# nyu-systems/Grendel-GS

Measured on NVIDIA H100. Metric: train-step Gaussians/s (preprocess+forward+loss+backward), higher is better.
Workload: dtype f32

## Files before the change

### grendel-gs_b200/csrc/binning.cu

```cuda
#include <cub/cub.cuh>

#include "common.cuh"
#include <atomic>
#include <cfloat>
#include <mutex>

#define BIN_THREADS 256

GS_D uint32_t count_local_tiles(int i, int W, int H, const float *__restrict__ means2D, const int32_t *__restrict__ radii,
                                const uint8_t *__restrict__ compute_locally, const GsViews &views) {
    const int gx = (W + GS_BLOCK_X - 1) / GS_BLOCK_X, gy = (H + GS_BLOCK_Y - 1) / GS_BLOCK_Y;
    const int r = radii[i];
    uint32_t n = 0;
    if (r > 0) {
        const float2 m = *reinterpret_cast<const float2 *>(means2D + 2 * i);
        int x0, y0, x1, y1;
        gs_get_rect(m.x, m.y, r, gx, gy, x0, y0, x1, y1);
        const uint8_t *mask = compute_locally + (size_t)gs_view_of(views, i) * views.T;
        for (int y = y0; y < y1; y++) {
            const uint8_t *row = mask + y * gx;
            for (int x = x0; x < x1; x++) n += row[x] ? 1u : 0u;
        }
    }
    return n;
}

__global__ void __launch_bounds__(BIN_THREADS)
k_count_tiles(int P, int W, int H, const float *__restrict__ means2D, const float *__restrict__ conic_opacity,
              const float *__restrict__ rgb, const float *__restrict__ depths, const int32_t *__restrict__ radii,
              const uint8_t *__restrict__ compute_locally, uint32_t *__restrict__ touched,
              uint32_t *__restrict__ depth_key, uint32_t *__restrict__ index, float *__restrict__ rec, int no_cull,
              unsigned long long *__restrict__ total64, const GsViews views) {
    const int i = blockIdx.x * BIN_THREADS + threadIdx.x;
    const bool valid = i < P;
    const uint32_t my_n = valid ? count_local_tiles(i, W, H, means2D, radii, compute_locally, views) : 0u;
    {
        __shared__ uint32_t s_sum[BIN_THREADS / 32];
        const uint32_t wsum = __reduce_add_sync(0xffffffffu, my_n);
        if ((threadIdx.x & 31) == 0) s_sum[threadIdx.x >> 5] = wsum;
        __syncthreads();
        if (threadIdx.x == 0) {
            unsigned long long t = 0ull;
#pragma unroll
            for (int w = 0; w < BIN_THREADS / 32; w++) t += s_sum[w];
            if (t) atomicAdd(total64, t);
        }
    }
    if (!valid) return;
    const uint32_t n = my_n;
    const float2 m = *reinterpret_cast<const float2 *>(means2D + 2 * i);
    touched[i] = n;
    depth_key[i] = n > 0 ? __float_as_uint(depths[i]) : 0xffffffffu;
    index[i] = (uint32_t)i;
    float4 r0 = make_float4(0.f, 0.f, 0.f, 0.f), r1 = r0, r2 = r0;
    if (n > 0) {
        const float4 co = *reinterpret_cast<const float4 *>(conic_opacity + 4 * i);
        const float thr = -logf(255.0f * fmaxf(co.w, 1e-30f));
        const float t = -2.f * thr;
        const float bb = co.y * co.y, bb_err = __fmaf_rn(co.y, co.y, -bb);
        const float det = __fmaf_rn(co.x, co.z, -bb) - bb_err;
        float ex = -1.f, ey = -1.f;
        if (t >= 0.f) {
            if (!no_cull && det >= FLT_MIN && co.x > 0.f && co.z > 0.f) {
                ex = sqrtf(t * co.z / det) * 1.02f + 0.5f;
                ey = sqrtf(t * co.x / det) * 1.02f + 0.5f;
            } else {
                ex = ey = 3.0e38f;
            }
        }
        r0 = make_float4(m.x, m.y, -0.5f * co.x, -co.y);
        r1 = make_float4(-0.5f * co.z, co.w, thr, rgb[3 * i]);
        r2 = make_float4(rgb[3 * i + 1], rgb[3 * i + 2], ex, ey);
    }
    float4 *o = reinterpret_cast<float4 *>(rec + (size_t)GS_REC_FLOATS * i);
    o[0] = r0; o[1] = r1; o[2] = r2;
}

struct TouchedInDepthOrder {
    const uint32_t *order, *touched;
    __host__ __device__ __forceinline__ uint32_t operator()(int s) const { return touched[order[s]]; }
};

template <bool DET>
__global__ void __launch_bounds__(BIN_THREADS)
k_duplicate(int P, int W, int H, const float *__restrict__ means2D, const int32_t *__restrict__ radii,
            const uint8_t *__restrict__ compute_locally, const uint32_t *__restrict__ order,
            const uint32_t *__restrict__ offsets, uint32_t *__restrict__ tile_keys, uint32_t *__restrict__ ids,
            const GsViews views, uint32_t *__restrict__ slots) {
    const int s = blockIdx.x * BIN_THREADS + threadIdx.x;
    if (s >= P) return;
    uint32_t off = (s == 0) ? 0u : offsets[s - 1];
    if (offsets[s] == off) return;
    const uint32_t i = order[s];
    const int gx = (W + GS_BLOCK_X - 1) / GS_BLOCK_X, gy = (H + GS_BLOCK_Y - 1) / GS_BLOCK_Y;
    const float2 m = *reinterpret_cast<const float2 *>(means2D + 2 * (size_t)i);
    int x0, y0, x1, y1;
    gs_get_rect(m.x, m.y, radii[i], gx, gy, x0, y0, x1, y1);
    const int t0 = gs_view_of(views, (int)i) * views.T;
    for (int y = y0; y < y1; y++)
        for (int x = x0; x < x1; x++) {
            const int t = t0 + y * gx + x;
            if (!compute_locally[t]) continue;
            tile_keys[off] = (uint32_t)t;
            ids[off] = i;
            if (DET) slots[off] = off;
            off++;
        }
}

__global__ void __launch_bounds__(BIN_THREADS)
k_gather_ids(int64_t R, const uint32_t *__restrict__ sorted_u, const uint32_t *__restrict__ ids_unsorted,
             uint32_t *__restrict__ ids_sorted) {
    const int64_t r = (int64_t)blockIdx.x * BIN_THREADS + threadIdx.x;
    if (r < R) ids_sorted[r] = __ldg(ids_unsorted + __ldg(sorted_u + r));
}

GS_D uint32_t lower_bound_u32(const uint32_t *__restrict__ keys, uint32_t n, uint32_t v) {
    uint32_t lo = 0, hi = n;
    while (lo < hi) {
        const uint32_t mid = lo + ((hi - lo) >> 1);
        if (__ldg(keys + mid) < v) lo = mid + 1; else hi = mid;
    }
    return lo;
}
__global__ void __launch_bounds__(BIN_THREADS)
k_tile_ranges(int64_t R, int T, const uint32_t *__restrict__ tile_keys, uint32_t *__restrict__ ranges) {
    const int t = blockIdx.x * BIN_THREADS + threadIdx.x;
    if (t >= T) return;
    const uint32_t a = lower_bound_u32(tile_keys, (uint32_t)R, (uint32_t)t);
    const uint32_t b = lower_bound_u32(tile_keys, (uint32_t)R, (uint32_t)t + 1u);
    reinterpret_cast<uint2 *>(ranges)[t] = a < b ? make_uint2(a, b) : make_uint2(0u, 0u);
}

static size_t align_up(size_t v, size_t a) { return (v + a - 1) / a * a; }

static size_t count_cub_bytes(int P) {
    size_t scan = 0, sort = 0;
    const int n = P > 0 ? P : 1;
    {
        cub::CountingInputIterator<int> idx(0);
        cub::TransformInputIterator<uint32_t, TouchedInDepthOrder, cub::CountingInputIterator<int>> in(
            idx, TouchedInDepthOrder{nullptr, nullptr});
        cub::DeviceScan::InclusiveSum(nullptr, scan, in, (uint32_t *)nullptr, n);
    }
    cub::DeviceRadixSort::SortPairs(nullptr, sort, (const uint32_t *)nullptr, (uint32_t *)nullptr,
                                    (const uint32_t *)nullptr, (uint32_t *)nullptr, n, 0, 32);
    return align_up(scan > sort ? scan : sort, 256);
}

extern "C" size_t gs_render_count_temp_bytes(int P) {
    return 5 * align_up((size_t)(P > 0 ? P : 1) * sizeof(uint32_t), 256) + count_cub_bytes(P) + 256;
}

static int make_views(int num_views, const int32_t *view_start, int T, GsViews &v) {
    GS_REQUIRE(num_views >= 1 && num_views <= GS_MAX_VIEWS, "num_views must be in [1, GS_MAX_VIEWS]");
    GS_REQUIRE(view_start != nullptr && view_start[0] == 0, "view_start[0] must be 0");
    GS_REQUIRE((long long)T * num_views < (1ll << 31), "too many tiles");
    v.n = num_views;
    v.T = T;
    for (int k = 0; k <= GS_MAX_VIEWS; k++) v.start[k] = view_start[k <= num_views ? k : num_views];
    for (int k = 0; k < num_views; k++) GS_REQUIRE(v.start[k] <= v.start[k + 1], "view_start must be non-decreasing");
    return GS_OK;
}

#define GS_COUNT_SLOTS 64
static unsigned long long *g_count_slots = nullptr;
static cudaEvent_t g_count_events[GS_COUNT_SLOTS];
static std::atomic<unsigned> g_count_next{0};
static std::mutex g_count_mutex;

static unsigned long long *count_slot() {
    {
        std::lock_guard<std::mutex> lock(g_count_mutex);
        if (!g_count_slots) {
            if (cudaHostAlloc((void **)&g_count_slots, GS_COUNT_SLOTS * sizeof(unsigned long long), cudaHostAllocDefault) != cudaSuccess) {
                g_count_slots = nullptr;
                return nullptr;
            }
            for (int i = 0; i < GS_COUNT_SLOTS; i++)
                if (cudaEventCreateWithFlags(&g_count_events[i], cudaEventDisableTiming) != cudaSuccess) {
                    cudaFreeHost(g_count_slots);
                    g_count_slots = nullptr;
                    return nullptr;
                }
        }
    }
    return g_count_slots + (g_count_next.fetch_add(1) % GS_COUNT_SLOTS);
}

extern "C" int gs_render_count_launch(int num_views, const int32_t *view_start, int P1, int image_height, int image_width,
                                      const float *means2D, const float *conic_opacity, const float *rgb,
                                      const float *depths, const int32_t *radii, const uint8_t *compute_locally,
                                      uint32_t *order, uint32_t *offsets, float *rec, void *temp, size_t temp_bytes,
                                      void **ticket, void *stream_) {
    cudaStream_t stream = (cudaStream_t)stream_;
    GS_REQUIRE(image_height > 0 && image_width > 0, "sizes");
    GS_REQUIRE(ticket != nullptr, "ticket");
    *ticket = nullptr;
    const int32_t one_view[2] = {0, P1};
    if (view_start == nullptr) {
        GS_REQUIRE(num_views == 1 && P1 >= 0, "view_start may only be NULL for one view");
        view_start = one_view;
    }
    GsViews views;
    {
        const int gx = (image_width + GS_BLOCK_X - 1) / GS_BLOCK_X, gy = (image_height + GS_BLOCK_Y - 1) / GS_BLOCK_Y;
        const int rc = make_views(num_views, view_start, gx * gy, views);
        if (rc != GS_OK) return rc;
    }
    const int P = views.start[num_views];
    unsigned long long *slot = count_slot();
    GS_REQUIRE(slot != nullptr, "pinned host slot for the instance count");
    *slot = 0ull;
    *ticket = slot;
    if (P == 0) {
        GS_CUDA_TRY(cudaEventRecord(g_count_events[slot - g_count_slots], stream));
        return GS_OK;
    }
    GS_REQUIRE(means2D && conic_opacity && rgb && depths && radii && compute_locally && order && offsets && rec && temp,
               "null pointer");
    GS_REQUIRE(((uintptr_t)rec & 15) == 0 && ((uintptr_t)conic_opacity & 15) == 0 && ((uintptr_t)means2D & 7) == 0,
               "alignment");
    if (temp_bytes < gs_render_count_temp_bytes(P)) {
        gs_set_error("gs_render_count: temp too small (%zu < %zu)", temp_bytes, gs_render_count_temp_bytes(P));
        return GS_ENOMEM;
    }
    const size_t stride = align_up((size_t)P * sizeof(uint32_t), 256);
    char *base = (char *)temp;
    uint32_t *touched = (uint32_t *)base, *dkey = (uint32_t *)(base + stride), *dkey_sorted = (uint32_t *)(base + 2 * stride),
             *index = (uint32_t *)(base + 3 * stride);
    void *cub_temp = base + 5 * stride;
    size_t cub_bytes = count_cub_bytes(P);
    unsigned long long *total64 = (unsigned long long *)(base + 5 * stride + cub_bytes);
    GS_CUDA_TRY(cudaMemsetAsync(total64, 0, sizeof(unsigned long long), stream));
    const int grid = (P + BIN_THREADS - 1) / BIN_THREADS;
    {
        GsStageTimer timer(GS_STAGE_COUNT_TILES, stream);
        k_count_tiles<<<grid, BIN_THREADS, 0, stream>>>(P, image_width, image_height, means2D, conic_opacity, rgb, depths,
                                                        radii, compute_locally, touched, dkey, index, rec,
                                                        (g_gs_debug_flags & GS_DEBUG_NO_BLOCK_CULL) ? 1 : 0, total64, views);
        GS_LAUNCH_CHECK();
    }
    GS_CUDA_TRY(cudaMemcpyAsync(slot, total64, sizeof(unsigned long long), cudaMemcpyDeviceToHost, stream));
    GS_CUDA_TRY(cudaEventRecord(g_count_events[slot - g_count_slots], stream));
    {
        GsStageTimer timer(GS_STAGE_SORT, stream);
        GS_CUDA_TRY(cub::DeviceRadixSort::SortPairs(cub_temp, cub_bytes, dkey, dkey_sorted, index, order, P, 0, 32, stream));
    }
    {
        GsStageTimer timer(GS_STAGE_SCAN, stream);
        cub::CountingInputIterator<int> idx(0);
        cub::TransformInputIterator<uint32_t, TouchedInDepthOrder, cub::CountingInputIterator<int>> in(
            idx, TouchedInDepthOrder{order, touched});
        GS_CUDA_TRY(cub::DeviceScan::InclusiveSum(cub_temp, cub_bytes, in, offsets, P, stream));
    }
    return GS_OK;
}

extern "C" int gs_render_count_read(void *ticket, int64_t *R_host, void *stream_) {
    GS_REQUIRE(ticket != nullptr && R_host != nullptr, "ticket / R_host");
    *R_host = 0;
    (void)stream_;
    const ptrdiff_t idx = (unsigned long long *)ticket - g_count_slots;
    GS_REQUIRE(g_count_slots != nullptr && idx >= 0 && idx < GS_COUNT_SLOTS, "not a ticket of gs_render_count_launch");
    GS_CUDA_TRY(cudaEventSynchronize(g_count_events[idx]));
    const unsigned long long total = *(volatile unsigned long long *)ticket;
    if (total >= (1ull << 31)) {
        gs_set_error("gs_render_count: %llu splat-tile instances in one call (limit 2^31 - 1): render fewer views per call",
                     total);
        return GS_EINVAL;
    }
    *R_host = (int64_t)total;
    return GS_OK;
}

extern "C" int gs_render_count_batched(int num_views, const int32_t *view_start, int image_height, int image_width,
                                       const float *means2D, const float *conic_opacity, const float *rgb,
                                       const float *depths, const int32_t *radii, const uint8_t *compute_locally,
                                       uint32_t *order, uint32_t *offsets, float *rec, void *temp, size_t temp_bytes,
                                       int64_t *R_host, void *stream_) {
    GS_REQUIRE(R_host != nullptr, "R_host");
    *R_host = 0;
    GS_REQUIRE(view_start != nullptr, "view_start[0] must be 0");
    void *ticket = nullptr;
    const int rc = gs_render_count_launch(num_views, view_start, 0, image_height, image_width, means2D, conic_opacity, rgb,
                                          depths, radii, compute_locally, order, offsets, rec, temp, temp_bytes, &ticket,
                                          stream_);
    if (rc != GS_OK) return rc;
    return gs_render_count_read(ticket, R_host, stream_);
}

extern "C" int gs_render_count(int P, int image_height, int image_width, const float *means2D,
                               const float *conic_opacity, const float *rgb, const float *depths, const int32_t *radii,
                               const uint8_t *compute_locally, uint32_t *order, uint32_t *offsets, float *rec,
                               void *temp, size_t temp_bytes, int64_t *R_host, void *stream) {
    GS_REQUIRE(P >= 0, "sizes");
    const int32_t one_view[2] = {0, P};
    return gs_render_count_batched(1, one_view, image_height, image_width, means2D, conic_opacity, rgb, depths, radii,
                                   compute_locally, order, offsets, rec, temp, temp_bytes, R_host, stream);
}

static int tile_bits(int T) {
    int b = 0;
    while ((1ll << b) < (long long)T) b++;
    return b > 0 ? b : 1;
}

extern "C" size_t gs_render_sort_temp_bytes(int64_t R) {
    size_t bytes = 0;
    cub::DeviceRadixSort::SortPairs(nullptr, bytes, (const uint32_t *)nullptr, (uint32_t *)nullptr,
                                    (const uint32_t *)nullptr, (uint32_t *)nullptr, R > 0 ? R : 1, 0, 32);
    return align_up(bytes, 256) + 256;
}

int gs_launch_blend_forward(int num_views, int64_t R, int H, int W, const float *rec, const float *bg,
                            const uint8_t *compute_locally, const uint32_t *ranges, const uint32_t *ids_sorted,
                            float *image, float *final_T, uint32_t *n_contrib, int64_t *stats, int64_t *tile_stats,
                            void *seg_ws, size_t seg_ws_bytes, cudaStream_t stream);

static int render_forward_impl(int num_views, const int32_t *view_start, int64_t R, int image_height, int image_width,
                               const float *means2D, const int32_t *radii, const uint8_t *compute_locally,
                               const uint32_t *order, const uint32_t *offsets, const float *rec, const float *bg,
                               uint32_t *tiles_unsorted, uint32_t *ids_unsorted, uint32_t *tiles_sorted,
                               uint32_t *ids_sorted, uint32_t *sorted_u, void *sort_temp, size_t sort_temp_bytes,
                               uint32_t *ranges, float *image, float *final_T, uint32_t *n_contrib, int64_t *stats,
                               int64_t *tile_stats, void *seg_ws, size_t seg_ws_bytes, cudaStream_t stream) {
    GS_REQUIRE(R >= 0 && image_height > 0 && image_width > 0, "sizes");
    GS_REQUIRE(R < (1ll << 31), "more than 2^31 splat-tile instances");
    GS_REQUIRE(compute_locally && bg && ranges && image && final_T && n_contrib, "null pointer");
    GS_REQUIRE(((uintptr_t)tile_stats & 7) == 0, "tile_stats must be 8-byte aligned");
    const int gx = (image_width + GS_BLOCK_X - 1) / GS_BLOCK_X, gy = (image_height + GS_BLOCK_Y - 1) / GS_BLOCK_Y;
    GsViews views;
    {
        const int rc = make_views(num_views, view_start, gx * gy, views);
        if (rc != GS_OK) return rc;
    }
    const int P = views.start[num_views];
    const int T = gx * gy * num_views;
    GS_REQUIRE(ranges != nullptr && ((uintptr_t)ranges & 7) == 0, "ranges must be 8-byte aligned");
    if (R == 0) GS_CUDA_TRY(cudaMemsetAsync(ranges, 0, sizeof(uint32_t) * 2 * (size_t)T, stream));
    if (R > 0) {
        GS_REQUIRE(means2D && radii && order && offsets && rec && tiles_unsorted && ids_unsorted && tiles_sorted &&
                       ids_sorted && sort_temp,
                   "null pointer");
        if (sort_temp_bytes < gs_render_sort_temp_bytes(R)) {
            gs_set_error("gs_render_forward: sort temp too small");
            return GS_ENOMEM;
        }
        if (!sorted_u) {
            {
                GsStageTimer timer(GS_STAGE_DUPLICATE, stream);
                k_duplicate<false><<<(P + BIN_THREADS - 1) / BIN_THREADS, BIN_THREADS, 0, stream>>>(
                    P, image_width, image_height, means2D, radii, compute_locally, order, offsets, tiles_unsorted,
                    ids_unsorted, views, nullptr);
                GS_LAUNCH_CHECK();
            }
            {
                GsStageTimer timer(GS_STAGE_SORT, stream);
                GS_CUDA_TRY(cub::DeviceRadixSort::SortPairs(sort_temp, sort_temp_bytes, tiles_unsorted, tiles_sorted,
                                                            ids_unsorted, ids_sorted, (int)R, 0, tile_bits(T), stream));
            }
        } else {
            {
                GsStageTimer timer(GS_STAGE_DUPLICATE, stream);
                k_duplicate<true><<<(P + BIN_THREADS - 1) / BIN_THREADS, BIN_THREADS, 0, stream>>>(
                    P, image_width, image_height, means2D, radii, compute_locally, order, offsets, tiles_unsorted,
                    ids_unsorted, views, ids_sorted);
                GS_LAUNCH_CHECK();
            }
            {
                GsStageTimer timer(GS_STAGE_SORT, stream);
                GS_CUDA_TRY(cub::DeviceRadixSort::SortPairs(sort_temp, sort_temp_bytes, tiles_unsorted, tiles_sorted,
                                                            ids_sorted, sorted_u, (int)R, 0, tile_bits(T), stream));
                k_gather_ids<<<(unsigned)((R + BIN_THREADS - 1) / BIN_THREADS), BIN_THREADS, 0, stream>>>(
                    R, sorted_u, ids_unsorted, ids_sorted);
                GS_LAUNCH_CHECK();
            }
        }
        {
            GsStageTimer timer(GS_STAGE_RANGES, stream);
            k_tile_ranges<<<(T + BIN_THREADS - 1) / BIN_THREADS, BIN_THREADS, 0, stream>>>(R, T, tiles_sorted, ranges);
            GS_LAUNCH_CHECK();
        }
    }
    return gs_launch_blend_forward(num_views, R, image_height, image_width, rec, bg, compute_locally, ranges, ids_sorted,
                                   image, final_T, n_contrib, stats, tile_stats, seg_ws, seg_ws_bytes, stream);
}

extern "C" int gs_render_forward_batched_ts(int num_views, const int32_t *view_start, int64_t R, int image_height,
                                            int image_width, const float *means2D, const int32_t *radii,
                                            const uint8_t *compute_locally, const uint32_t *order, const uint32_t *offsets,
                                            const float *rec, const float *bg, uint32_t *tiles_unsorted,
                                            uint32_t *ids_unsorted, uint32_t *tiles_sorted, uint32_t *ids_sorted,
                                            void *sort_temp, size_t sort_temp_bytes, uint32_t *ranges, float *image,
                                            float *final_T, uint32_t *n_contrib, int64_t *stats, int64_t *tile_stats,
                                            void *seg_ws, size_t seg_ws_bytes, void *stream) {
    return render_forward_impl(num_views, view_start, R, image_height, image_width, means2D, radii, compute_locally, order,
                               offsets, rec, bg, tiles_unsorted, ids_unsorted, tiles_sorted, ids_sorted, nullptr, sort_temp,
                               sort_temp_bytes, ranges, image, final_T, n_contrib, stats, tile_stats, seg_ws, seg_ws_bytes,
                               (cudaStream_t)stream);
}

extern "C" int gs_render_forward_det(int num_views, const int32_t *view_start, int P, int64_t R, int image_height,
                                     int image_width, const float *means2D, const int32_t *radii,
                                     const uint8_t *compute_locally, const uint32_t *order, const uint32_t *offsets,
                                     const float *rec, const float *bg, uint32_t *tiles_unsorted, uint32_t *ids_unsorted,
                                     uint32_t *tiles_sorted, uint32_t *ids_sorted, uint32_t *sorted_u, void *sort_temp,
                                     size_t sort_temp_bytes, uint32_t *ranges, float *image, float *final_T,
                                     uint32_t *n_contrib, int64_t *stats, int64_t *tile_stats, void *seg_ws,
                                     size_t seg_ws_bytes, void *stream) {
    const int32_t one_view[2] = {0, P};
    if (view_start == nullptr) {
        GS_REQUIRE(num_views == 1 && P >= 0, "view_start may only be NULL for one view");
        view_start = one_view;
    }
    GS_REQUIRE(R == 0 || (sorted_u != nullptr && ids_unsorted != nullptr && ids_sorted != nullptr), "null pointer");
    GS_REQUIRE(((uintptr_t)sorted_u & 3) == 0 && ((uintptr_t)ids_unsorted & 3) == 0 && ((uintptr_t)ids_sorted & 3) == 0,
               "instance arrays must be 4-byte aligned");
    return render_forward_impl(num_views, view_start, R, image_height, image_width, means2D, radii, compute_locally, order,
                               offsets, rec, bg, tiles_unsorted, ids_unsorted, tiles_sorted, ids_sorted,
                               R > 0 ? sorted_u : nullptr, sort_temp, sort_temp_bytes, ranges, image, final_T, n_contrib,
                               stats, tile_stats, seg_ws, seg_ws_bytes, (cudaStream_t)stream);
}

extern "C" int gs_render_forward_batched(int num_views, const int32_t *view_start, int64_t R, int image_height,
                                         int image_width, const float *means2D, const int32_t *radii,
                                         const uint8_t *compute_locally, const uint32_t *order, const uint32_t *offsets,
                                         const float *rec, const float *bg, uint32_t *tiles_unsorted,
                                         uint32_t *ids_unsorted, uint32_t *tiles_sorted, uint32_t *ids_sorted,
                                         void *sort_temp, size_t sort_temp_bytes, uint32_t *ranges, float *image,
                                         float *final_T, uint32_t *n_contrib, int64_t *stats, void *seg_ws,
                                         size_t seg_ws_bytes, void *stream) {
    return gs_render_forward_batched_ts(num_views, view_start, R, image_height, image_width, means2D, radii,
                                        compute_locally, order, offsets, rec, bg, tiles_unsorted, ids_unsorted,
                                        tiles_sorted, ids_sorted, sort_temp, sort_temp_bytes, ranges, image, final_T,
                                        n_contrib, stats, nullptr, seg_ws, seg_ws_bytes, stream);
}

extern "C" int gs_render_forward_ts(int P, int64_t R, int image_height, int image_width, const float *means2D,
                                    const int32_t *radii, const uint8_t *compute_locally, const uint32_t *order,
                                    const uint32_t *offsets, const float *rec, const float *bg, uint32_t *tiles_unsorted,
                                    uint32_t *ids_unsorted, uint32_t *tiles_sorted, uint32_t *ids_sorted, void *sort_temp,
                                    size_t sort_temp_bytes, uint32_t *ranges, float *image, float *final_T,
                                    uint32_t *n_contrib, int64_t *stats, int64_t *tile_stats, void *seg_ws,
                                    size_t seg_ws_bytes, void *stream) {
    GS_REQUIRE(P >= 0, "sizes");
    const int32_t one_view[2] = {0, P};
    return gs_render_forward_batched_ts(1, one_view, R, image_height, image_width, means2D, radii, compute_locally,
                                        order, offsets, rec, bg, tiles_unsorted, ids_unsorted, tiles_sorted, ids_sorted,
                                        sort_temp, sort_temp_bytes, ranges, image, final_T, n_contrib, stats, tile_stats,
                                        seg_ws, seg_ws_bytes, stream);
}

extern "C" int gs_render_forward(int P, int64_t R, int image_height, int image_width, const float *means2D,
                                 const int32_t *radii, const uint8_t *compute_locally, const uint32_t *order,
                                 const uint32_t *offsets, const float *rec, const float *bg, uint32_t *tiles_unsorted,
                                 uint32_t *ids_unsorted, uint32_t *tiles_sorted, uint32_t *ids_sorted, void *sort_temp,
                                 size_t sort_temp_bytes, uint32_t *ranges, float *image, float *final_T,
                                 uint32_t *n_contrib, int64_t *stats, void *seg_ws, size_t seg_ws_bytes, void *stream) {
    return gs_render_forward_ts(P, R, image_height, image_width, means2D, radii, compute_locally, order, offsets, rec, bg,
                                tiles_unsorted, ids_unsorted, tiles_sorted, ids_sorted, sort_temp, sort_temp_bytes, ranges,
                                image, final_T, n_contrib, stats, nullptr, seg_ws, seg_ws_bytes, stream);
}
```

Measured before the change: 596.5 million.

## Spread each warp's splat-tile duplication across lanes with cooperative ballot compaction

Rewrites k_duplicate so each warp scans its 32 Gaussians' bounding-box areas and processes all tile cells in 32-wide chunks. Each lane binary-searches for its owning Gaussian via shuffles and writes local tiles at ballot/popc-compacted offsets. This replaces the per-thread serial loops and removes divergence from uneven footprints, making the stores coalesced and contiguous. The cost is extra shuffles and integer div/mod per cell, plus a new guard on tiles per view. It also adds profiling and equivalence-check scripts.

Result: slower. 571.2 million, median of 6 (-4.2%).

```diff
diff --git a/grendel-gs_b200/csrc/binning.cu b/grendel-gs_b200/csrc/binning.cu
--- a/grendel-gs_b200/csrc/binning.cu
+++ b/grendel-gs_b200/csrc/binning.cu
@@ -88,24 +88,58 @@
             const uint32_t *__restrict__ offsets, uint32_t *__restrict__ tile_keys, uint32_t *__restrict__ ids,
             const GsViews views, uint32_t *__restrict__ slots) {
     const int s = blockIdx.x * BIN_THREADS + threadIdx.x;
-    if (s >= P) return;
-    uint32_t off = (s == 0) ? 0u : offsets[s - 1];
-    if (offsets[s] == off) return;
-    const uint32_t i = order[s];
+    const int lane = threadIdx.x & 31;
+    if (s - lane >= P) return;
     const int gx = (W + GS_BLOCK_X - 1) / GS_BLOCK_X, gy = (H + GS_BLOCK_Y - 1) / GS_BLOCK_Y;
-    const float2 m = *reinterpret_cast<const float2 *>(means2D + 2 * (size_t)i);
-    int x0, y0, x1, y1;
-    gs_get_rect(m.x, m.y, radii[i], gx, gy, x0, y0, x1, y1);
-    const int t0 = gs_view_of(views, (int)i) * views.T;
-    for (int y = y0; y < y1; y++)
-        for (int x = x0; x < x1; x++) {
-            const int t = t0 + y * gx + x;
-            if (!compute_locally[t]) continue;
+    uint32_t first_slot = 0u, area = 0u, id = 0u;
+    int x0 = 0, y0 = 0, w = 1, t0 = 0;
+    if (s < P) {
+        first_slot = (s == 0) ? 0u : offsets[s - 1];
+        if (offsets[s] != first_slot) {
+            id = order[s];
+            const float2 m = *reinterpret_cast<const float2 *>(means2D + 2 * (size_t)id);
+            int x1, y1;
+            gs_get_rect(m.x, m.y, radii[id], gx, gy, x0, y0, x1, y1);
+            w = x1 - x0;
+            area = (uint32_t)(w * (y1 - y0));
+            t0 = gs_view_of(views, (int)id) * views.T;
+        }
+    }
+    uint32_t incl = area;
+#pragma unroll
+    for (int d = 1; d < 32; d <<= 1) {
+        const uint32_t o = __shfl_up_sync(0xffffffffu, incl, d);
+        if (lane >= d) incl += o;
+    }
+    const uint32_t first_cell = incl - area, total = __shfl_sync(0xffffffffu, incl, 31);
+    const uint32_t base = __shfl_sync(0xffffffffu, first_slot, 0);
+    const uint32_t lt = (1u << lane) - 1u;
+    uint32_t done = 0u;
+    for (uint32_t b = 0; b < total; b += 32) {
+        const uint32_t k = b + (uint32_t)lane;
+        int j = 0;
+#pragma unroll
+        for (int step = 16; step > 0; step >>= 1)
+            if (__shfl_sync(0xffffffffu, first_cell, j + step) <= k) j += step;
+        const uint32_t f = __shfl_sync(0xffffffffu, first_cell, j), sid = __shfl_sync(0xffffffffu, id, j);
+        const int rx = __shfl_sync(0xffffffffu, x0, j), ry = __shfl_sync(0xffffffffu, y0, j);
+        const int rw = __shfl_sync(0xffffffffu, w, j), rt = __shfl_sync(0xffffffffu, t0, j);
+        bool local = false;
+        int t = 0;
+        if (k < total) {
+            const uint32_t c = k - f;
+            t = rt + (ry + (int)(c / (uint32_t)rw)) * gx + rx + (int)(c % (uint32_t)rw);
+            local = compute_locally[t] != 0;
+        }
+        const uint32_t ball = __ballot_sync(0xffffffffu, local);
+        if (local) {
+            const uint32_t off = base + done + __popc(ball & lt);
             tile_keys[off] = (uint32_t)t;
-            ids[off] = i;
+            ids[off] = sid;
             if (DET) slots[off] = off;
-            off++;
-        }
+        }
+        done += __popc(ball);
+    }
 }
 
 __global__ void __launch_bounds__(BIN_THREADS)
@@ -338,6 +372,7 @@
     const int P = views.start[num_views];
     const int T = gx * gy * num_views;
     GS_REQUIRE(ranges != nullptr && ((uintptr_t)ranges & 7) == 0, "ranges must be 8-byte aligned");
+    GS_REQUIRE((long long)gx * gy * 32 < (1ll << 32), "too many tiles per view");
     if (R == 0) GS_CUDA_TRY(cudaMemsetAsync(ranges, 0, sizeof(uint32_t) * 2 * (size_t)T, stream));
     if (R > 0) {
         GS_REQUIRE(means2D && radii && order && offsets && rec && tiles_unsorted && ids_unsorted && tiles_sorted &&
diff --git a/profiles/binning_compare.py b/profiles/binning_compare.py
--- /dev/null
+++ b/profiles/binning_compare.py
@@ -0,0 +1,68 @@
+import argparse
+import os
+import subprocess
+import sys
+
+import numpy as np
+
+KEYS = ("ids", "sorted_u", "ranges", "image", "final_T", "n_contrib", "g_means2D", "g_conic_opacity", "g_rgb",
+        "d_image", "d_final_T", "d_n_contrib", "d_ranges", "d_ids")
+
+
+def worker(tree, out):
+    sys.path[:0] = [tree, os.path.join(tree, "grendel-gs_b200"), os.path.join(tree, "tests")]
+    import torch
+    import det_util as du
+    import gpu_util as gu
+    from gs_b200 import _lib, synthetic as syn
+    _lib.load()
+    W, H = 1920, 1080
+    sc = syn.make_scene(2_000_000, W, H, seed=0)
+    cam = syn.make_camera(W, H, yaw_deg=2.0)
+    pre, _, _ = gu.preprocess_forward(sc, cam)
+    T = ((H + 15) // 16) * ((W + 15) // 16)
+    cl = torch.ones((T,), dtype=torch.uint8, device=gu.DEV)
+    views = [(pre["means2D"], pre["conic_opacity"], pre["rgb"], pre["depths"], pre["radii"], cl)]
+    f = du.forward(views, H, W, [0.0, 0.0, 0.0], det=True)
+    R = f["R"]
+    dL = gu.to_dev(np.random.default_rng(3).standard_normal((1, 3, H, W)).astype(np.float32))
+    g = du.backward(f, dL, det=True)
+    d = du.forward(views, H, W, [0.0, 0.0, 0.0], det=False)
+    res = dict(ids=f["ids"][:R], sorted_u=f["sorted_u"][:R], ranges=f["ranges"], image=f["image"], final_T=f["final_T"],
+               n_contrib=f["n_contrib"], g_means2D=g["means2D"], g_conic_opacity=g["conic_opacity"], g_rgb=g["rgb"],
+               d_image=d["image"], d_final_T=d["final_T"], d_n_contrib=d["n_contrib"], d_ranges=d["ranges"],
+               d_ids=d["ids"][:R])
+    os.makedirs(out, exist_ok=True)
+    for k, v in res.items():
+        np.save(os.path.join(out, k + ".npy"), v.detach().cpu().numpy())
+    print(f"R = {R}")
+
+
+def main():
+    ap = argparse.ArgumentParser()
+    ap.add_argument("--trees", nargs=2)
+    ap.add_argument("--out", default="runs/binning_compare")
+    ap.add_argument("--worker", nargs=2, metavar=("TREE", "OUT"))
+    a = ap.parse_args()
+    if a.worker:
+        worker(os.path.abspath(a.worker[0]), a.worker[1])
+        return
+    dirs = []
+    for k, tree in enumerate(a.trees):
+        d = os.path.join(a.out, f"tree{k}")
+        p = subprocess.run([sys.executable, os.path.abspath(__file__), "--worker", tree, d], capture_output=True, text=True)
+        print(tree, p.stdout.strip(), p.stderr[-3000:] if p.returncode else "")
+        if p.returncode:
+            raise SystemExit("worker failed")
+        dirs.append(d)
+    ok = True
+    for k in KEYS:
+        x, y = (np.load(os.path.join(d, k + ".npy")) for d in dirs)
+        same = x.shape == y.shape and x.tobytes() == y.tobytes()
+        ok &= same
+        print(f"{k:18s} {'identical' if same else 'DIFFERENT'} {x.shape}")
+    print("ALL IDENTICAL" if ok else "DIFFERENCES FOUND")
+
+
+if __name__ == "__main__":
+    main()
diff --git a/profiles/binning_timing.py b/profiles/binning_timing.py
--- /dev/null
+++ b/profiles/binning_timing.py
@@ -0,0 +1,104 @@
+import argparse
+import json
+import os
+import subprocess
+import sys
+
+BINNING = ("k_count_tiles", "k_duplicate", "k_gather_ids", "k_tile_ranges")
+
+
+def label(name):
+    for key in BINNING:
+        if key in name:
+            return key
+    if "Radix" in name or "Onesweep" in name:
+        return "radix"
+    if "Scan" in name:
+        return "cub scan"
+    return None
+
+
+def worker(tree, B, steps, warmup):
+    sys.path[:0] = [tree, os.path.join(tree, "grendel-gs_b200")]
+    import torch
+    from torch.profiler import ProfilerActivity, profile
+    import bench
+    from gs_b200 import _lib, ops
+    _lib.load()
+    args = argparse.Namespace(workload="c2", n=0)
+    cfg = bench.workload(args)
+    tr = bench.build_trainer(args, cfg, B, torch.device("cuda", 0), 0, 1)
+    for _ in range(warmup):
+        tr.step(resident=True)
+    torch.cuda.synchronize()
+    with profile(activities=[ProfilerActivity.CUDA]) as prof:
+        for _ in range(steps):
+            tr.step(resident=True)
+        torch.cuda.synchronize()
+    R = max(ops._R_HINT.values())
+    rows = {}
+    radix = []
+    for ev in prof.events():
+        if ev.device_type != torch.autograd.DeviceType.CUDA:
+            continue
+        lab = label(ev.name)
+        if lab is None:
+            continue
+        if lab == "radix":
+            radix.append((ev.time_range.start, ev.device_time, ev.name))
+            continue
+        rows[lab] = rows.get(lab, 0.0) + ev.device_time
+    radix.sort()
+    per_step = len(radix) // steps if steps else 0
+    depth_kernels = per_step // 2 if "k_duplicate" in rows else per_step
+    for k, (_, dt, _) in enumerate(radix):
+        lab = "radix, depth" if (k % per_step) < depth_kernels else "radix, tile"
+        rows[lab] = rows.get(lab, 0.0) + dt
+    out = {k: v / steps / 1000.0 for k, v in rows.items()}
+    return dict(tree=tree, B=B, R=R, P=tr.P if hasattr(tr, "P") else None, ms=out)
+
+
+def main():
+    ap = argparse.ArgumentParser()
+    ap.add_argument("--trees", nargs="+", required=True)
+    ap.add_argument("--views", nargs="+", type=int, default=[1, 4])
+    ap.add_argument("--rounds", type=int, default=2)
+    ap.add_argument("--steps", type=int, default=20)
+    ap.add_argument("--warmup", type=int, default=5)
+    ap.add_argument("--out", default=None)
+    ap.add_argument("--worker", nargs=2, metavar=("TREE", "B"))
+    a = ap.parse_args()
+    if a.worker:
+        print("RESULT " + json.dumps(worker(os.path.abspath(a.worker[0]), int(a.worker[1]), a.steps, a.warmup)))
+        return
+    gpu = subprocess.run(["nvidia-smi", "--query-gpu=name,power.limit,clocks.max.sm", "--format=csv,noheader"],
+                         capture_output=True, text=True).stdout.strip()
+    print("gpu:", gpu)
+    res = []
+    for r in range(a.rounds):
+        for B in a.views:
+            for tree in a.trees:
+                p = subprocess.run([sys.executable, os.path.abspath(__file__), "--trees", tree, "--worker", tree, str(B),
+                                    "--steps", str(a.steps), "--warmup", str(a.warmup)], capture_output=True, text=True)
+                line = [x for x in p.stdout.splitlines() if x.startswith("RESULT ")]
+                if p.returncode or not line:
+                    print(p.stdout[-2000:], p.stderr[-4000:])
+                    raise SystemExit(f"worker failed: {tree} B={B}")
+                d = json.loads(line[0][7:])
+                d["round"] = r
+                res.append(d)
+                chain = sum(v for k, v in d["ms"].items() if k not in ("k_count_tiles", "radix, depth", "cub scan"))
+                print(f"round {r} B={B} {tree}: R={d['R']} chain(after scan)={chain:.4f} ms  " +
+                      "  ".join(f"{k}={v:.4f}" for k, v in sorted(d["ms"].items())))
+                T = 120 * 68 * B
+                need = 8 * d["R"] + 8 * T
+                print(f"    chain bytes {need / 1e6:.1f} MB -> {need / (chain * 1e-3) / 1e12:.2f} TB/s "
+                      f"({100 * need / (chain * 1e-3) / 3.35e12:.1f} % of 3.35 TB/s)")
+    if a.out:
+        os.makedirs(os.path.dirname(a.out) or ".", exist_ok=True)
+        with open(a.out, "w") as f:
+            json.dump(dict(gpu=gpu, results=res), f, indent=1)
+
+
+if __name__ == "__main__":
+    main()
```
